# deepspeedai/DeepSpeed

Measured on AMD Instinct MI355X. Metric: tokens/sec Llama-3-8B ZeRO-3, higher is better.
Workload: dtype bf16; 1 GPU; model=llama3-8b, global_batch=8, seq_len=4096, parallelism=zero3_dp1, grad_accum=2

## Files before the change

deepspeed_amd/ops/csrc/attention.hip:

```cpp
#include <torch/extension.h>

#include "common.h"

using bf16x8_t = __attribute__((ext_vector_type(8))) short;

constexpr int KVTILE = 64;
constexpr int VT_PAD = 8;

DEV_INLINE int vtswz(int d, int kv_byte) {
  return d * ((KVTILE + VT_PAD) * 2) + (kv_byte ^ (((d >> 5) & 3) << 5));
}


using f32x16_t = __attribute__((ext_vector_type(16))) float;
#define MFMA_BF16_32x32x16 __builtin_amdgcn_mfma_f32_32x32x16_bf16

constexpr int QB5 = 32;
constexpr int QT5 = 256;
constexpr int KT5 = 64;

DEV_INLINE float half_swap(float x, int hi) {
  int i = __builtin_bit_cast(int, x);
  auto r = __builtin_amdgcn_permlane32_swap(i, i, false, false);
  return __builtin_bit_cast(float, hi ? r[0] : r[1]);
}

DEV_INLINE unsigned int cvtpk2(float lo, float hi) {
  unsigned short a = __builtin_bit_cast(unsigned short, (__bf16)lo);
  unsigned short b = __builtin_bit_cast(unsigned short, (__bf16)hi);
  return (unsigned int)a | ((unsigned int)b << 16);
}

template <int DH>
DEV_INLINE int kswz_t(int row, int byte_off) {
  return row * (DH * 2) + (byte_off ^ ((row & 7) << 4));
}

template <int DH>
__launch_bounds__(512, 2)
__global__ void flash_fwd_v5_kernel(
    const short* __restrict__ q,
    const short* __restrict__ k,
    const short* __restrict__ v,
    short* __restrict__ out,
    float* __restrict__ lse_out,
    const float* __restrict__ kvmask,
    int B, int S, int Hq, int Hk, float scale, int causal) {
  __shared__ short k_lds[2][KT5 * DH];
  __shared__ short vt_lds[DH * (KT5 + VT_PAD)];

  const int lane = threadIdx.x & 63;
  const int wave = threadIdx.x >> 6;
  const int l31 = lane & 31;
  const int hi = lane >> 5;

  constexpr int NQF = DH / 16;
  constexpr int NOT = DH / 32;

  const int qtile = blockIdx.x;
  const int bh = blockIdx.y;
  const int b = bh / Hq;
  const int h = bh % Hq;
  const int hk = h / (Hq / Hk);
  const int qbase = qtile * QT5;
  const int wave_q = qbase + wave * QB5;
  const int my_q = wave_q + l31;

  const long long qrs = (long long)Hq * DH;
  const long long kvrs = (long long)Hk * DH;
  const short* qp = q + ((long long)b * S) * qrs + h * DH;
  const short* kp = k + ((long long)b * S) * kvrs + hk * DH;
  const short* vp = v + ((long long)b * S) * kvrs + hk * DH;
  const float* mp = kvmask ? kvmask + (long long)b * S : nullptr;

  bf16x8_t qfrag[NQF];
  {
    int srow = my_q < S ? my_q : S - 1;
    const short* src = qp + (long long)srow * qrs + hi * 8;
#pragma unroll
    for (int ks = 0; ks < NQF; ++ks)
      qfrag[ks] = *reinterpret_cast<const bf16x8_t*>(src + 16 * ks);
  }

  const float sc2 = scale * 1.44269504f;
  float m_run = -INFINITY, l_run = 0.f;
  f32x16_t ot[NOT];
#pragma unroll
  for (int mt = 0; mt < NOT; ++mt)
#pragma unroll
    for (int r = 0; r < 16; ++r) ot[mt][r] = 0.f;

  const int kv_end = causal ? min(S, qbase + QT5) : S;
  const int n_tiles = (kv_end + KT5 - 1) / KT5;

  constexpr int VTPR = DH / 16;
  const int st_row = threadIdx.x / VTPR;
  const int st_c0 = (threadIdx.x % VTPR) * 16;
  constexpr int KSEGS = KT5 * DH * 2 / 1024;
  constexpr int KPASSES = (KSEGS + 7) / 8;

#define ISSUE_K(t_)                                                          \
  {                                                                          \
    int kvb_ = (t_)*KT5;                                                     \
    short* kbuf_ = k_lds[(t_)&1];                                            \
    for (int pass = 0; pass < KPASSES; ++pass) {                             \
      int seg = pass * 8 + wave;                                             \
      int linear = seg * 1024 + lane * 16;                                   \
      int row = linear / (DH * 2);                                           \
      int colbyte = linear % (DH * 2);                                       \
      int src_col = colbyte ^ ((row & 7) << 4);                              \
      int grow = kvb_ + row;                                                 \
      int srow = grow < S ? grow : S - 1;                                    \
      const short* src = kp + (long long)srow * kvrs + (src_col >> 1);       \
      __builtin_amdgcn_global_load_lds(                                      \
          reinterpret_cast<const unsigned int*>(src),                        \
          reinterpret_cast<unsigned int*>(reinterpret_cast<char*>(kbuf_) +   \
                                          seg * 1024),                       \
          16, 0, 0);                                                         \
    }                                                                        \
  }

#define LOAD_V(t_, dst_)                                                     \
  {                                                                          \
    int grow = (t_)*KT5 + st_row;                                            \
    const short* vrow = vp + (long long)grow * kvrs;                         \
    if (st_row < KT5 && grow < S) {                                          \
      dst_[0] = *reinterpret_cast<const bf16x8_t*>(vrow + st_c0);            \
      dst_[1] = *reinterpret_cast<const bf16x8_t*>(vrow + st_c0 + 8);        \
    } else {                                                                 \
      dst_[0] = bf16x8_t{0, 0, 0, 0, 0, 0, 0, 0};                            \
      dst_[1] = bf16x8_t{0, 0, 0, 0, 0, 0, 0, 0};                            \
    }                                                                        \
  }

  bf16x8_t vreg[2], vnext[2];
  ISSUE_K(0);
  LOAD_V(0, vreg);

  for (int t = 0; t < n_tiles; ++t) {
    const int kvbase = t * KT5;
    const bool has_next = (t + 1) < n_tiles;
    if (has_next) ISSUE_K(t + 1);
    if (st_row < KT5) {
      char* vbase = reinterpret_cast<char*>(vt_lds);
#pragma unroll
      for (int cc = 0; cc < 2; ++cc) {
        int col = st_c0 + cc * 8;
#pragma unroll
        for (int j = 0; j < 8; ++j)
          *reinterpret_cast<short*>(vbase + vtswz(col + j, st_row * 2)) =
              vreg[cc][j];
      }
    }
    if (has_next) LOAD_V(t + 1, vnext);
    __syncthreads();

    f32x16_t st[2];
    __builtin_amdgcn_s_setprio(1);
#pragma unroll
    for (int mt = 0; mt < 2; ++mt) {
      f32x16_t acc;
#pragma unroll
      for (int r = 0; r < 16; ++r) acc[r] = 0.f;
      int krow = 32 * mt + l31;
#pragma unroll
      for (int ks = 0; ks < NQF; ++ks) {
        bf16x8_t kf = *reinterpret_cast<const bf16x8_t*>(
            reinterpret_cast<char*>(k_lds[t & 1]) +
            kswz_t<DH>(krow, (16 * ks + hi * 8) * 2));
        acc = MFMA_BF16_32x32x16(kf, qfrag[ks], acc, 0, 0, 0);
      }
      st[mt] = acc;
    }
    __builtin_amdgcn_s_setprio(0);

    const bool btile = (causal && (kvbase + KT5 > qbase)) ||
                       (kvbase + KT5 > S) || mp != nullptr;
    float tmax = -INFINITY;
    if (btile) {
#pragma unroll
      for (int mt = 0; mt < 2; ++mt)
#pragma unroll
        for (int r = 0; r < 16; ++r) {
          float sv = st[mt][r] * sc2;
          int gkv = kvbase + 32 * mt + (r & 3) + 8 * (r >> 2) + 4 * hi;
          if (mp && gkv < S) sv += mp[gkv] * 1.44269504f;
          if ((causal && gkv > my_q) || gkv >= S) sv = -INFINITY;
          st[mt][r] = sv;
          tmax = fmaxf(tmax, sv);
        }
    } else {
#pragma unroll
      for (int mt = 0; mt < 2; ++mt)
#pragma unroll
        for (int r = 0; r < 16; ++r) {
          float sv = st[mt][r] * sc2;
          st[mt][r] = sv;
          tmax = fmaxf(tmax, sv);
        }
    }
    tmax = fmaxf(tmax, half_swap(tmax, hi));
    if (!__all(tmax - m_run <= 11.5416f)) {
      float m_new = fmaxf(m_run, tmax);
      float c = (m_run == -INFINITY) ? 0.f : __builtin_amdgcn_exp2f(m_run - m_new);
      l_run *= c;
#pragma unroll
      for (int mt = 0; mt < NOT; ++mt)
#pragma unroll
        for (int r = 0; r < 16; ++r) ot[mt][r] *= c;
      m_run = m_new;
    }
    float m_sub = m_run;
    if (btile) m_sub = (m_run == -INFINITY) ? 0.f : m_run;
    float psum = 0.f;
#pragma unroll
    for (int mt = 0; mt < 2; ++mt)
#pragma unroll
      for (int r = 0; r < 16; ++r) {
        float p = __builtin_amdgcn_exp2f(st[mt][r] - m_sub);
        st[mt][r] = p;
        psum += p;
      }
    psum += half_swap(psum, hi);
    l_run += psum;

    bf16x8_t pfrag[4];
#pragma unroll
    for (int ks = 0; ks < 4; ++ks) {
      int mt = ks >> 1, s = ks & 1;
      unsigned int wA0 = cvtpk2(st[mt][8 * s + 0], st[mt][8 * s + 1]);
      unsigned int wA1 = cvtpk2(st[mt][8 * s + 2], st[mt][8 * s + 3]);
      unsigned int wB0 = cvtpk2(st[mt][8 * s + 4], st[mt][8 * s + 5]);
      unsigned int wB1 = cvtpk2(st[mt][8 * s + 6], st[mt][8 * s + 7]);
      auto r0 = __builtin_amdgcn_permlane32_swap((int)wA0, (int)wB0,
                                                 false, false);
      auto r1 = __builtin_amdgcn_permlane32_swap((int)wA1, (int)wB1,
                                                 false, false);
      unsigned int w[4] = {(unsigned int)r0[0], (unsigned int)r1[0],
                           (unsigned int)r0[1], (unsigned int)r1[1]};
      pfrag[ks] = *reinterpret_cast<bf16x8_t*>(w);
    }

    __builtin_amdgcn_s_setprio(1);
#pragma unroll
    for (int mt = 0; mt < NOT; ++mt) {
      int drow = 32 * mt + l31;
#pragma unroll
      for (int ks = 0; ks < 4; ++ks) {
        bf16x8_t vf = *reinterpret_cast<const bf16x8_t*>(
            reinterpret_cast<char*>(vt_lds) +
            vtswz(drow, (16 * ks + hi * 8) * 2));
        ot[mt] = MFMA_BF16_32x32x16(vf, pfrag[ks], ot[mt], 0, 0, 0);
      }
    }
    __builtin_amdgcn_s_setprio(0);
    __syncthreads();
    vreg[0] = vnext[0];
    vreg[1] = vnext[1];
  }
#undef ISSUE_K
#undef LOAD_V

  if (my_q < S) {
    float inv_l = (l_run > 0.f) ? 1.f / l_run : 0.f;
    short* orow = out + ((long long)b * S + my_q) * qrs + h * DH;
#pragma unroll
    for (int mt = 0; mt < NOT; ++mt)
#pragma unroll
      for (int g = 0; g < 4; ++g) {
        int d0 = 32 * mt + 8 * g + 4 * hi;
        unsigned int w[2];
        w[0] = cvtpk2(ot[mt][4 * g + 0] * inv_l, ot[mt][4 * g + 1] * inv_l);
        w[1] = cvtpk2(ot[mt][4 * g + 2] * inv_l, ot[mt][4 * g + 3] * inv_l);
        *reinterpret_cast<unsigned long long*>(orow + d0) =
            *reinterpret_cast<unsigned long long*>(w);
      }
    if (hi == 0 && lse_out)
      lse_out[((long long)b * Hq + h) * S + my_q] =
          0.693147181f * (m_run + __log2f(fmaxf(l_run, 1e-30f)));
  }
}

void flash_check_qkv(const at::Tensor& q, const at::Tensor& k,
                     const at::Tensor& v, const char* who) {
  CHECK_ARG(q, at::kBFloat16);
  CHECK_ARG(k, at::kBFloat16);
  CHECK_ARG(v, at::kBFloat16);
  CHECK_ON(k, q);
  CHECK_ON(v, q);
  TORCH_CHECK(q.dim() == 4 && k.dim() == 4 && v.dim() == 4, who,
              ": q, k, v must be [B,S,H,D]");
  const long D = q.size(3);
  TORCH_CHECK(D == 128 || D == 64, who, ": head_dim must be 64 or 128");
  TORCH_CHECK(q.size(1) >= 1 && q.size(2) >= 1 && k.size(2) >= 1, who,
              ": empty sequence or head dimension");
  TORCH_CHECK(k.size(0) == q.size(0) && k.size(1) == q.size(1) &&
                  k.size(3) == D,
              who, ": k must be [B,S,Hk,D] with q's B, S and D");
  TORCH_CHECK(v.sizes() == k.sizes(), who, ": v must have k's shape");
  TORCH_CHECK(q.size(2) % k.size(2) == 0, who, ": GQA requires Hq % Hk == 0");
}

const float* flash_check_kvmask(const c10::optional<at::Tensor>& kvmask,
                                const at::Tensor& q) {
  if (!kvmask.has_value() || !kvmask->defined()) return nullptr;
  TORCH_CHECK(kvmask->is_cuda() && kvmask->device() == q.device() &&
                  kvmask->scalar_type() == at::kFloat &&
                  kvmask->is_contiguous() &&
                  kvmask->numel() == q.size(0) * q.size(1),
              "kvmask must be a contiguous float [B,S] tensor on q's device");
  return kvmask->data_ptr<float>();
}

std::vector<at::Tensor> flash_attn_fwd(at::Tensor q, at::Tensor k,
                                       at::Tensor v, bool causal,
                                       double scale,
                                       c10::optional<at::Tensor> kvmask) {
  flash_check_qkv(q, k, v, "flash_attn_fwd");
  int B = q.size(0), S = q.size(1), Hq = q.size(2), D = q.size(3);
  int Hk = k.size(2);
  const float* mp = flash_check_kvmask(kvmask, q);
  const float fscale =
      scale == 0.0 ? 1.0f / std::sqrt((float)D) : (float)scale;
  auto out = at::empty_like(q);
  auto lse = at::empty({B, Hq, S}, q.options().dtype(at::kFloat));
  auto stream = c10::hip::getCurrentHIPStream();
  dim3 grid((S + QT5 - 1) / QT5, B * Hq);
  if (D == 128) {
    hipLaunchKernelGGL(flash_fwd_v5_kernel<128>, grid, dim3(512), 0,
                       stream.stream(),
                       reinterpret_cast<const short*>(q.data_ptr()),
                       reinterpret_cast<const short*>(k.data_ptr()),
                       reinterpret_cast<const short*>(v.data_ptr()),
                       reinterpret_cast<short*>(out.data_ptr()),
                       lse.data_ptr<float>(), mp, B, S, Hq, Hk, fscale,
                       causal ? 1 : 0);
  } else {
    hipLaunchKernelGGL(flash_fwd_v5_kernel<64>, grid, dim3(512), 0,
                       stream.stream(),
                       reinterpret_cast<const short*>(q.data_ptr()),
                       reinterpret_cast<const short*>(k.data_ptr()),
                       reinterpret_cast<const short*>(v.data_ptr()),
                       reinterpret_cast<short*>(out.data_ptr()),
                       lse.data_ptr<float>(), mp, B, S, Hq, Hk, fscale,
                       causal ? 1 : 0);
  }
  HIP_CHECK_KERNEL();
  return {out, lse};
}
```

deepspeed_amd/ops/csrc/attention_bwd.hip:

```cpp
#include <torch/extension.h>

#include "common.h"
#include "flash_bwd_layout.h"

using bf16x8_t = __attribute__((ext_vector_type(8))) short;
using f32x4_t = __attribute__((ext_vector_type(4))) float;
using u32x4_t = __attribute__((ext_vector_type(4))) unsigned int;
using u32x2_t = __attribute__((ext_vector_type(2))) unsigned int;

#define MFMA_BF16_16x16x32 __builtin_amdgcn_mfma_f32_16x16x32_bf16

namespace bwd {

constexpr int BR = 128;
constexpr int WR = 32;
constexpr int KTW1 = 1;
constexpr int TS = 32;
static_assert(TS == bwd_layout::TS, "the image layout is for 32-row steps");
constexpr int PT = 64;

DEV_INLINE unsigned int cvtpk2(float lo, float hi) {
  unsigned short a = __builtin_bit_cast(unsigned short, (__bf16)lo);
  unsigned short b = __builtin_bit_cast(unsigned short, (__bf16)hi);
  return (unsigned int)a | ((unsigned int)b << 16);
}

template <int DH>
__launch_bounds__(256)
__global__ void bwd_preprocess(
    const short* __restrict__ dout, const short* __restrict__ out,
    const float* __restrict__ lse,
    float* __restrict__ drowP, float* __restrict__ lseP,
    int B, int S, int Sp, int Hq) {
  constexpr int PPR = DH / 8;
  const int bh = blockIdx.y;
  const int b = bh / Hq;
  const int h = bh % Hq;
  const int s0 = blockIdx.x * PT;

  for (int i = threadIdx.x; i < PT * PPR; i += 256) {
    const int row = i / PPR;
    const int c = i % PPR;
    const int s = s0 + row;
    const long long off = (((long long)b * S + s) * Hq + h) * DH + c * 8;
    u32x4_t x = {0u, 0u, 0u, 0u};
    u32x4_t o = {0u, 0u, 0u, 0u};
    if (s < S) {
      x = *reinterpret_cast<const u32x4_t*>(dout + off);
      o = *reinterpret_cast<const u32x4_t*>(out + off);
    }
    float acc = 0.f;
#pragma unroll
    for (int w = 0; w < 4; ++w)
      acc += bf2f((short)(x[w] & 0xffff)) * bf2f((short)(o[w] & 0xffff)) +
             bf2f((short)(x[w] >> 16)) * bf2f((short)(o[w] >> 16));
#pragma unroll
    for (int m = PPR / 2; m > 0; m >>= 1) acc += __shfl_xor(acc, m, WAVE);
    if (c == 0) {
      float l = 0.f;
      if (s < S) {
        l = lse[((long long)b * Hq + h) * S + s];
        if (l == -INFINITY) l = INFINITY;
      }
      drowP[((long long)b * Hq + h) * Sp + s] = acc;
      lseP[((long long)b * Hq + h) * Sp + s] = l;
    }
  }
}

DEV_INLINE void lds_dma16(const short* src, char* lds_wave_base) {
  __builtin_amdgcn_global_load_lds(
      reinterpret_cast<const unsigned int*>(src),
      reinterpret_cast<unsigned int*>(lds_wave_base), 16, 0, 0);
}

template <int DH>
DEV_INLINE void issue_rm(const short* base, long long rs, int r0, int S,
                         char* img, int sseg, int lane) {
  const int linear = sseg * 1024 + lane * 16;
  const int src_col = bwd_layout::dma_src_byte<DH>(linear);
  const int grow = r0 + bwd_layout::dma_row<DH>(linear);
  const int srow = grow < S ? grow : S - 1;
  lds_dma16(base + (long long)srow * rs + (src_col >> 1), img + sseg * 1024);
}

template <int DH>
DEV_INLINE bf16x8_t read_rm(const char* img, int row, int ks, int l4) {
  return *reinterpret_cast<const bf16x8_t*>(
      img + bwd_layout::img_off<DH>(row, (l4 * 8 + 32 * ks) * 2));
}

DEV_INLINE unsigned lds_addr(const char* p) {
  return (unsigned)(size_t)(
      (const __attribute__((address_space(3))) char*)p);
}

struct tr_frag {
  u32x2_t lo, hi;
};

template <int DH>
DEV_INLINE tr_frag issue_tr_read(unsigned img, int dt, int lane) {
  tr_frag f;
  const unsigned a0 = img + bwd_layout::tr_read_addr<DH>(lane, dt, 0);
  const unsigned a1 = img + bwd_layout::tr_read_addr<DH>(lane, dt, 1);
  asm volatile("ds_read_b64_tr_b16 %0, %1" : "=v"(f.lo) : "v"(a0) : "memory");
  asm volatile("ds_read_b64_tr_b16 %0, %1" : "=v"(f.hi) : "v"(a1) : "memory");
  return f;
}

template <int N>
DEV_INLINE void tr_wait(tr_frag& a, tr_frag& b) {
  asm volatile("s_waitcnt lgkmcnt(%4)"
               : "+v"(a.lo), "+v"(a.hi), "+v"(b.lo), "+v"(b.hi)
               : "n"(N));
}

template <int N>
DEV_INLINE void tr_wait(tr_frag& a) {
  asm volatile("s_waitcnt lgkmcnt(%2)" : "+v"(a.lo), "+v"(a.hi) : "n"(N));
}

DEV_INLINE bf16x8_t tr_operand(const tr_frag& f) {
  u32x4_t w = {f.lo[0], f.lo[1], f.hi[0], f.hi[1]};
  return __builtin_bit_cast(bf16x8_t, w);
}

DEV_INLINE bf16x8_t pack_pair(const f32x4_t& a, const f32x4_t& b) {
  u32x4_t w = {cvtpk2(a[0], a[1]), cvtpk2(a[2], a[3]), cvtpk2(b[0], b[1]),
               cvtpk2(b[2], b[3])};
  return __builtin_bit_cast(bf16x8_t, w);
}

DEV_INLINE void store4(short* p, const f32x4_t& a) {
  u32x2_t w = {cvtpk2(a[0], a[1]), cvtpk2(a[2], a[3])};
  *reinterpret_cast<u32x2_t*>(p) = w;
}

template <int NDT, int STRIDE>
DEV_INLINE void unrotate_row(f32x4_t* acc ,
                             const float* __restrict__ cr,
                             const float* __restrict__ sr) {
#pragma unroll
  for (int dt = 0; dt < NDT / 2; ++dt) {
    const f32x4_t c = *reinterpret_cast<const f32x4_t*>(cr + 16 * dt);
    const f32x4_t sn = *reinterpret_cast<const f32x4_t*>(sr + 16 * dt);
    const f32x4_t d1 = acc[dt * STRIDE];
    const f32x4_t d2 = acc[(dt + NDT / 2) * STRIDE];
    acc[dt * STRIDE] = d1 * c + d2 * sn;
    acc[(dt + NDT / 2) * STRIDE] = d2 * c - d1 * sn;
  }
}

template <int DH, int KTW, bool ROPE>
__launch_bounds__(512 / KTW, 1)
__global__ void flash_bwd_dkv_kernel(
    const short* __restrict__ q,
    const short* __restrict__ k,
    const short* __restrict__ v,
    const short* __restrict__ dout,
    const float* __restrict__ lseP,
    const float* __restrict__ drowP,
    const float* __restrict__ kvmask,
    short* __restrict__ dk,
    short* __restrict__ dv,
    const float* __restrict__ rope_cos,
    const float* __restrict__ rope_sin,
    int B, int S, int Sp, int Hq, int Hk, float scale, int causal) {
  constexpr int NKS = DH / 32;
  constexpr int NDT = DH / 16;
  constexpr int IMG = TS * DH * 2;
  constexpr int SPI = DH / 16;
  constexpr int NW = 8 / KTW;
  constexpr int WRK = 16 * KTW;
  constexpr int LD_OFF = 2 * IMG;
  constexpr int BUF = LD_OFF + 256;
  __shared__ __attribute__((aligned(16))) char smem[2 * BUF];

  const int lane = threadIdx.x & 63;
  const int wave = __builtin_amdgcn_readfirstlane(threadIdx.x >> 6);
  const int l15 = lane & 15;
  const int l4 = lane >> 4;

  const int bh = blockIdx.y;
  const int b = bh / Hk;
  const int hk = bh % Hk;
  const int G = Hq / Hk;
  const int kv_base = blockIdx.x * BR;
  const int wk = kv_base + wave * WRK;

  const long long qrs = (long long)Hq * DH;
  const long long kvrs = (long long)Hk * DH;
  const short* kp = k + ((long long)b * S) * kvrs + hk * DH;
  const short* vp = v + ((long long)b * S) * kvrs + hk * DH;

  bf16x8_t kfrag[KTW][NKS], vfrag[KTW][NKS];
  float maskv[KTW];
#pragma unroll
  for (int kt = 0; kt < KTW; ++kt) {
    const int krow = wk + 16 * kt + l15;
    const int srow = krow < S ? krow : S - 1;
    const short* ks = kp + (long long)srow * kvrs;
    const short* vs = vp + (long long)srow * kvrs;
#pragma unroll
    for (int ks_i = 0; ks_i < NKS; ++ks_i) {
      kfrag[kt][ks_i] =
          *reinterpret_cast<const bf16x8_t*>(ks + ks_i * 32 + l4 * 8);
      vfrag[kt][ks_i] =
          *reinterpret_cast<const bf16x8_t*>(vs + ks_i * 32 + l4 * 8);
    }
    maskv[kt] = (kvmask && krow < S) ? kvmask[(long long)b * S + krow] : 0.f;
  }
#pragma unroll
  for (int kt = 0; kt < KTW; ++kt) {
#pragma unroll
    for (int ks_i = 0; ks_i < NKS; ++ks_i) {
      asm volatile("" : "+v"(kfrag[kt][ks_i]));
      asm volatile("" : "+v"(vfrag[kt][ks_i]));
    }
    asm volatile("" : "+v"(maskv[kt]));
  }

  f32x4_t dk_acc[NDT][KTW], dv_acc[NDT][KTW];
#pragma unroll
  for (int dt = 0; dt < NDT; ++dt)
#pragma unroll
    for (int kt = 0; kt < KTW; ++kt) {
      dk_acc[dt][kt] = f32x4_t{0.f, 0.f, 0.f, 0.f};
      dv_acc[dt][kt] = f32x4_t{0.f, 0.f, 0.f, 0.f};
    }

  const int q_start = causal ? kv_base : 0;
  const int nq = (S - q_start + TS - 1) / TS;
  const int total = G * nq;

  static_assert(SPI <= NW, "one image segment per wave at the most");
  auto issue = [&](int g, int qb, int bufi) {
    const int h = hk * G + g;
    char* buf = smem + bufi * BUF;
    const short* qp = q + ((long long)b * S) * qrs + h * DH;
    const short* dop = dout + ((long long)b * S) * qrs + h * DH;
    const long long roff = ((long long)b * Hq + h) * Sp;
    if (wave < SPI) {
      issue_rm<DH>(qp, qrs, qb, S, buf, wave, lane);
      issue_rm<DH>(dop, qrs, qb, S, buf + IMG, wave, lane);
    }
    if (wave == 0) {
      const float* s = (lane < 32 ? lseP : drowP) + roff + qb + (lane & 31);
      __builtin_amdgcn_global_load_lds(
          reinterpret_cast<const unsigned int*>(s),
          reinterpret_cast<unsigned int*>(buf + LD_OFF), 4, 0, 0);
    }
  };

  int g_nx = 0, qb_nx = q_start;
  issue(g_nx, qb_nx, 0);
  for (int it = 0; it < total; ++it) {
    const int qb = qb_nx;
    asm volatile("s_waitcnt vmcnt(0)" ::: "memory");
    __builtin_amdgcn_s_barrier();
    asm volatile("" ::: "memory");
    qb_nx += TS;
    if (qb_nx >= S) {
      qb_nx = q_start;
      ++g_nx;
    }
    if (it + 1 < total) issue(g_nx, qb_nx, (it + 1) & 1);

    if (wk >= S || (causal && qb + TS - 1 < wk)) continue;
    const bool interior = !kvmask && qb + TS <= S && wk + WRK <= S &&
                          (!causal || qb >= wk + WRK - 1);
    const char* buf = smem + (it & 1) * BUF;
    const float* ld = reinterpret_cast<const float*>(buf + LD_OFF);

    f32x4_t s_acc[2][KTW], dp_acc[2][KTW], lrow[2];
#pragma unroll
    for (int qt = 0; qt < 2; ++qt) {
      lrow[qt] = *reinterpret_cast<const f32x4_t*>(ld + 16 * qt + 4 * l4);
      f32x4_t dr = *reinterpret_cast<const f32x4_t*>(ld + 32 + 16 * qt + 4 * l4);
#pragma unroll
      for (int kt = 0; kt < KTW; ++kt) {
        s_acc[qt][kt] = f32x4_t{0.f, 0.f, 0.f, 0.f};
        dp_acc[qt][kt] = -dr;
      }
    }
    __builtin_amdgcn_s_setprio(1);
#pragma unroll
    for (int qt = 0; qt < 2; ++qt)
#pragma unroll
      for (int ks_i = 0; ks_i < NKS; ++ks_i) {
        bf16x8_t aq = read_rm<DH>(buf, l15 + 16 * qt, ks_i, l4);
        bf16x8_t ad = read_rm<DH>(buf + IMG, l15 + 16 * qt, ks_i, l4);
#pragma unroll
        for (int kt = 0; kt < KTW; ++kt) {
          s_acc[qt][kt] = MFMA_BF16_16x16x32(aq, kfrag[kt][ks_i],
                                             s_acc[qt][kt], 0, 0, 0);
          dp_acc[qt][kt] = MFMA_BF16_16x16x32(ad, vfrag[kt][ks_i],
                                              dp_acc[qt][kt], 0, 0, 0);
        }
      }
    __builtin_amdgcn_s_setprio(0);

    if (interior) {
#pragma unroll
      for (int qt = 0; qt < 2; ++qt)
#pragma unroll
        for (int kt = 0; kt < KTW; ++kt)
#pragma unroll
          for (int r = 0; r < 4; ++r) {
            float p = __expf(s_acc[qt][kt][r] * scale - lrow[qt][r]);
            s_acc[qt][kt][r] = p;
            dp_acc[qt][kt][r] = p * dp_acc[qt][kt][r] * scale;
          }
    } else {
#pragma unroll
      for (int qt = 0; qt < 2; ++qt)
#pragma unroll
        for (int kt = 0; kt < KTW; ++kt) {
          const int gkv = wk + 16 * kt + l15;
#pragma unroll
          for (int r = 0; r < 4; ++r) {
            const int gq = qb + 16 * qt + 4 * l4 + r;
            const bool valid = gq < S && gkv < S && (!causal || gq >= gkv);
            float sval = s_acc[qt][kt][r] * scale + maskv[kt];
            float p = valid ? __expf(sval - lrow[qt][r]) : 0.f;
            s_acc[qt][kt][r] = p;
            dp_acc[qt][kt][r] = p * dp_acc[qt][kt][r] * scale;
          }
        }
    }
    bf16x8_t pb[KTW], dsb[KTW];
#pragma unroll
    for (int kt = 0; kt < KTW; ++kt) {
      pb[kt] = pack_pair(s_acc[0][kt], s_acc[1][kt]);
      dsb[kt] = pack_pair(dp_acc[0][kt], dp_acc[1][kt]);
    }

    const unsigned qimg = lds_addr(buf);
    tr_frag fq[2], fd[2];
    fq[0] = issue_tr_read<DH>(qimg, 0, lane);
    fd[0] = issue_tr_read<DH>(qimg + IMG, 0, lane);
    __builtin_amdgcn_s_setprio(1);
#pragma unroll
    for (int dt = 0; dt < NDT; ++dt) {
      if (dt + 1 < NDT) {
        fq[(dt + 1) & 1] = issue_tr_read<DH>(qimg, dt + 1, lane);
        fd[(dt + 1) & 1] = issue_tr_read<DH>(qimg + IMG, dt + 1, lane);
        tr_wait<4>(fq[dt & 1], fd[dt & 1]);
      } else {
        tr_wait<0>(fq[dt & 1], fd[dt & 1]);
      }
      const bf16x8_t aqt = tr_operand(fq[dt & 1]);
      const bf16x8_t adt = tr_operand(fd[dt & 1]);
#pragma unroll
      for (int kt = 0; kt < KTW; ++kt) {
        dv_acc[dt][kt] =
            MFMA_BF16_16x16x32(adt, pb[kt], dv_acc[dt][kt], 0, 0, 0);
        dk_acc[dt][kt] =
            MFMA_BF16_16x16x32(aqt, dsb[kt], dk_acc[dt][kt], 0, 0, 0);
      }
    }
    __builtin_amdgcn_s_setprio(0);
  }

#pragma unroll
  for (int kt = 0; kt < KTW; ++kt) {
    const int gkv = wk + 16 * kt + l15;
    if (gkv >= S) continue;
    short* dkr = dk + ((long long)b * S + gkv) * kvrs + hk * DH + 4 * l4;
    short* dvr = dv + ((long long)b * S + gkv) * kvrs + hk * DH + 4 * l4;
    if (ROPE)
      unrotate_row<NDT, KTW>(&dk_acc[0][kt],
                             rope_cos + (long long)gkv * (DH / 2) + 4 * l4,
                             rope_sin + (long long)gkv * (DH / 2) + 4 * l4);
#pragma unroll
    for (int dt = 0; dt < NDT; ++dt) {
      store4(dkr + 16 * dt, dk_acc[dt][kt]);
      store4(dvr + 16 * dt, dv_acc[dt][kt]);
    }
  }
}

template <int DH, bool ROPE>
__launch_bounds__(256, 2)
__global__ void flash_bwd_dq_kernel(
    const short* __restrict__ q, const short* __restrict__ k,
    const short* __restrict__ v, const short* __restrict__ dout,
    const float* __restrict__ lseP,
    const float* __restrict__ drowP,
    const float* __restrict__ kvmask,
    short* __restrict__ dq,
    const float* __restrict__ rope_cos,
    const float* __restrict__ rope_sin,
    int B, int S, int Sp, int Hq, int Hk, float scale, int causal) {
  constexpr int NKS = DH / 32;
  constexpr int NDT = DH / 16;
  constexpr int IMG = TS * DH * 2;
  constexpr int SPI = DH / 16;
  constexpr int IPI = SPI / 4;
  constexpr int BUF = 2 * IMG;
  __shared__ __attribute__((aligned(16))) char smem[2 * BUF];

  const int lane = threadIdx.x & 63;
  const int wave = threadIdx.x >> 6;
  const int l15 = lane & 15;
  const int l4 = lane >> 4;

  const int qtile = gridDim.x - 1 - blockIdx.x;
  const int bh = blockIdx.y;
  const int b = bh / Hq;
  const int h = bh % Hq;
  const int hk = h / (Hq / Hk);
  const int qbase = qtile * BR;
  const int wq = qbase + wave * WR;

  const long long qrs = (long long)Hq * DH;
  const long long kvrs = (long long)Hk * DH;
  const short* qp = q + ((long long)b * S) * qrs + h * DH;
  const short* dop = dout + ((long long)b * S) * qrs + h * DH;
  const short* kp = k + ((long long)b * S) * kvrs + hk * DH;
  const short* vp = v + ((long long)b * S) * kvrs + hk * DH;
  const float* mp = kvmask ? kvmask + (long long)b * S : nullptr;

  bf16x8_t qfrag[2][NKS], dofrag[2][NKS];
  float lse_l[2], dr_l[2];
#pragma unroll
  for (int qt = 0; qt < 2; ++qt) {
    const int qrow = wq + 16 * qt + l15;
    const int srow = qrow < S ? qrow : S - 1;
    const short* qs = qp + (long long)srow * qrs;
    const short* ds = dop + (long long)srow * qrs;
#pragma unroll
    for (int ks_i = 0; ks_i < NKS; ++ks_i) {
      qfrag[qt][ks_i] =
          *reinterpret_cast<const bf16x8_t*>(qs + ks_i * 32 + l4 * 8);
      dofrag[qt][ks_i] =
          *reinterpret_cast<const bf16x8_t*>(ds + ks_i * 32 + l4 * 8);
    }
    lse_l[qt] = lseP[((long long)b * Hq + h) * Sp + qrow];
    dr_l[qt] = drowP[((long long)b * Hq + h) * Sp + qrow];
  }

  f32x4_t dq_acc[NDT][2];
#pragma unroll
  for (int dt = 0; dt < NDT; ++dt)
#pragma unroll
    for (int qt = 0; qt < 2; ++qt) dq_acc[dt][qt] = f32x4_t{0.f, 0.f, 0.f, 0.f};

  const int kv_end = causal ? min(S, qbase + BR) : S;
  const int n_tiles = (kv_end + TS - 1) / TS;

  auto issue = [&](int kvb, int bufi) {
    char* buf = smem + bufi * BUF;
#pragma unroll
    for (int i = 0; i < IPI; ++i) {
      const int sseg = i * 4 + wave;
      issue_rm<DH>(kp, kvrs, kvb, S, buf, sseg, lane);
      issue_rm<DH>(vp, kvrs, kvb, S, buf + IMG, sseg, lane);
    }
  };

  issue(0, 0);
  for (int t = 0; t < n_tiles; ++t) {
    const int kvb = t * TS;
    asm volatile("s_waitcnt vmcnt(0)" ::: "memory");
    __syncthreads();
    if (t + 1 < n_tiles) issue(kvb + TS, (t + 1) & 1);

    if (wq >= S || (causal && kvb > wq + WR - 1)) continue;
    const bool interior = !mp && kvb + TS <= S && wq + WR <= S &&
                          (!causal || kvb + TS - 1 <= wq);
    const char* buf = smem + (t & 1) * BUF;

    f32x4_t s_acc[2][2], dp_acc[2][2];
#pragma unroll
    for (int kt = 0; kt < 2; ++kt)
#pragma unroll
      for (int qt = 0; qt < 2; ++qt) {
        s_acc[kt][qt] = f32x4_t{0.f, 0.f, 0.f, 0.f};
        dp_acc[kt][qt] =
            f32x4_t{-dr_l[qt], -dr_l[qt], -dr_l[qt], -dr_l[qt]};
      }
    __builtin_amdgcn_s_setprio(1);
#pragma unroll
    for (int kt = 0; kt < 2; ++kt)
#pragma unroll
      for (int ks_i = 0; ks_i < NKS; ++ks_i) {
        bf16x8_t ak = read_rm<DH>(buf, l15 + 16 * kt, ks_i, l4);
        bf16x8_t av = read_rm<DH>(buf + IMG, l15 + 16 * kt, ks_i, l4);
#pragma unroll
        for (int qt = 0; qt < 2; ++qt) {
          s_acc[kt][qt] = MFMA_BF16_16x16x32(ak, qfrag[qt][ks_i],
                                             s_acc[kt][qt], 0, 0, 0);
          dp_acc[kt][qt] = MFMA_BF16_16x16x32(av, dofrag[qt][ks_i],
                                              dp_acc[kt][qt], 0, 0, 0);
        }
      }
    __builtin_amdgcn_s_setprio(0);

    if (interior) {
#pragma unroll
      for (int kt = 0; kt < 2; ++kt)
#pragma unroll
        for (int qt = 0; qt < 2; ++qt)
#pragma unroll
          for (int r = 0; r < 4; ++r) {
            float p = __expf(s_acc[kt][qt][r] * scale - lse_l[qt]);
            dp_acc[kt][qt][r] = p * dp_acc[kt][qt][r] * scale;
          }
    } else {
#pragma unroll
      for (int kt = 0; kt < 2; ++kt)
#pragma unroll
        for (int r = 0; r < 4; ++r) {
          const int gkv = kvb + 16 * kt + 4 * l4 + r;
          const float mv = (mp && gkv < S) ? mp[gkv] : 0.f;
#pragma unroll
          for (int qt = 0; qt < 2; ++qt) {
            const int gq = wq + 16 * qt + l15;
            const bool valid = gq < S && gkv < S && (!causal || gkv <= gq);
            float sval = s_acc[kt][qt][r] * scale + mv;
            float p = valid ? __expf(sval - lse_l[qt]) : 0.f;
            dp_acc[kt][qt][r] = p * dp_acc[kt][qt][r] * scale;
          }
        }
    }
    bf16x8_t dsb[2];
#pragma unroll
    for (int qt = 0; qt < 2; ++qt)
      dsb[qt] = pack_pair(dp_acc[0][qt], dp_acc[1][qt]);

    const unsigned kimg = lds_addr(buf);
    tr_frag fk[2];
    fk[0] = issue_tr_read<DH>(kimg, 0, lane);
    __builtin_amdgcn_s_setprio(1);
#pragma unroll
    for (int dt = 0; dt < NDT; ++dt) {
      if (dt + 1 < NDT) {
        fk[(dt + 1) & 1] = issue_tr_read<DH>(kimg, dt + 1, lane);
        tr_wait<2>(fk[dt & 1]);
      } else {
        tr_wait<0>(fk[dt & 1]);
      }
      const bf16x8_t akt = tr_operand(fk[dt & 1]);
#pragma unroll
      for (int qt = 0; qt < 2; ++qt)
        dq_acc[dt][qt] =
            MFMA_BF16_16x16x32(akt, dsb[qt], dq_acc[dt][qt], 0, 0, 0);
    }
    __builtin_amdgcn_s_setprio(0);
  }

#pragma unroll
  for (int qt = 0; qt < 2; ++qt) {
    const int gq = wq + 16 * qt + l15;
    if (gq >= S) continue;
    short* dqr = dq + ((long long)b * S + gq) * qrs + h * DH + 4 * l4;
    if (ROPE)
      unrotate_row<NDT, 2>(&dq_acc[0][qt],
                           rope_cos + (long long)gq * (DH / 2) + 4 * l4,
                           rope_sin + (long long)gq * (DH / 2) + 4 * l4);
#pragma unroll
    for (int dt = 0; dt < NDT; ++dt) store4(dqr + 16 * dt, dq_acc[dt][qt]);
  }
}

}

template <int DH, bool ROPE>
static void launch_bwd(at::Tensor& q, at::Tensor& k, at::Tensor& v,
                       at::Tensor& dout, at::Tensor& out, at::Tensor& lse,
                       at::Tensor& dq, at::Tensor& dk, at::Tensor& dv,
                       const float* mp, const float* cosp, const float* sinp,
                       int B, int S, int Hq, int Hk, float scale,
                       int causal) {
  auto stream = c10::hip::getCurrentHIPStream();
  const int Sp = (S + bwd::BR - 1) / bwd::BR * bwd::BR;
  auto drow = at::empty({B, Hq, Sp}, q.options().dtype(at::kFloat));
  auto lseP = at::empty({B, Hq, Sp}, q.options().dtype(at::kFloat));
  auto sp = [](const at::Tensor& t) {
    return reinterpret_cast<const short*>(t.data_ptr());
  };
  auto spm = [](at::Tensor& t) {
    return reinterpret_cast<short*>(t.data_ptr());
  };
  dim3 grid0(Sp / bwd::PT, B * Hq);
  hipLaunchKernelGGL(bwd::bwd_preprocess<DH>, grid0, dim3(256), 0,
                     stream.stream(), sp(dout), sp(out),
                     lse.data_ptr<float>(), drow.data_ptr<float>(),
                     lseP.data_ptr<float>(), B, S, Sp, Hq);
  HIP_CHECK_KERNEL();
  dim3 grid1(Sp / bwd::BR, B * Hk);
  hipLaunchKernelGGL((bwd::flash_bwd_dkv_kernel<DH, bwd::KTW1, ROPE>), grid1,
                     dim3(512 / bwd::KTW1), 0, stream.stream(), sp(q), sp(k),
                     sp(v), sp(dout), lseP.data_ptr<float>(),
                     drow.data_ptr<float>(), mp, spm(dk), spm(dv), cosp, sinp,
                     B, S, Sp, Hq, Hk, scale, causal);
  HIP_CHECK_KERNEL();
  dim3 grid2(Sp / bwd::BR, B * Hq);
  hipLaunchKernelGGL((bwd::flash_bwd_dq_kernel<DH, ROPE>), grid2, dim3(256), 0,
                     stream.stream(), sp(q), sp(k), sp(v), sp(dout),
                     lseP.data_ptr<float>(), drow.data_ptr<float>(), mp,
                     spm(dq), cosp, sinp, B, S, Sp, Hq, Hk, scale, causal);
  HIP_CHECK_KERNEL();
}

void flash_check_qkv(const at::Tensor& q, const at::Tensor& k,
                     const at::Tensor& v, const char* who);
const float* flash_check_kvmask(const c10::optional<at::Tensor>& kvmask,
                                const at::Tensor& q);
void check_rope_table(const at::Tensor& cos, const at::Tensor& sin,
                      const at::Tensor& ref, long long S, int D,
                      const char* who);

std::vector<at::Tensor> flash_attn_bwd(at::Tensor q, at::Tensor k,
                                       at::Tensor v, at::Tensor dout,
                                       at::Tensor out, at::Tensor lse,
                                       bool causal, double scale,
                                       c10::optional<at::Tensor> kvmask,
                                       c10::optional<at::Tensor> cos,
                                       c10::optional<at::Tensor> sin) {
  flash_check_qkv(q, k, v, "flash_attn_bwd");
  CHECK_ARG(dout, at::kBFloat16);
  CHECK_ARG(out, at::kBFloat16);
  CHECK_ARG(lse, at::kFloat);
  CHECK_ON(dout, q);
  CHECK_ON(out, q);
  CHECK_ON(lse, q);
  TORCH_CHECK(dout.sizes() == q.sizes() && out.sizes() == q.sizes(),
              "flash_attn_bwd: dout and out must have q's shape");
  int B = q.size(0), S = q.size(1), Hq = q.size(2), D = q.size(3);
  int Hk = k.size(2);
  TORCH_CHECK(lse.dim() == 3 && lse.size(0) == B && lse.size(1) == Hq &&
                  lse.size(2) == S,
              "flash_attn_bwd: lse must be [B,Hq,S]");
  const float* mp = flash_check_kvmask(kvmask, q);
  const float fscale =
      scale == 0.0 ? 1.0f / std::sqrt((float)D) : (float)scale;
  auto dq = at::empty_like(q);
  auto dk = at::empty_like(k);
  auto dv = at::empty_like(v);
  TORCH_CHECK(cos.has_value() == sin.has_value(),
              "flash_attn_bwd: cos and sin must be given together");
  const bool rope = cos.has_value();
  const float* cosp = nullptr;
  const float* sinp = nullptr;
  if (rope) {
    check_rope_table(*cos, *sin, q, S, D, "flash_attn_bwd");
    cosp = cos->data_ptr<float>();
    sinp = sin->data_ptr<float>();
  }
  const int ic = causal ? 1 : 0;
#define DSAMD_LAUNCH_BWD(DH_, ROPE_)                                        \
  launch_bwd<DH_, ROPE_>(q, k, v, dout, out, lse, dq, dk, dv, mp, cosp, sinp, \
                         B, S, Hq, Hk, fscale, ic)
  if (D == 128) {
    if (rope) DSAMD_LAUNCH_BWD(128, true); else DSAMD_LAUNCH_BWD(128, false);
  } else {
    if (rope) DSAMD_LAUNCH_BWD(64, true); else DSAMD_LAUNCH_BWD(64, false);
  }
#undef DSAMD_LAUNCH_BWD
  return {dq, dk, dv};
}
```

Measured before the change: 18220 tokens/s.

## Stage V via async LDS DMA and transpose-read it for forward attention

The forward flash-attention kernel no longer loads V into registers and scatters it into a transposed LDS buffer element by element. V now goes in row-major through global_load_lds DMA, double-buffered alongside K, and is read with ds_read_b64_tr_b16 transposing loads that are software-pipelined against the PV MFMAs. The second __syncthreads per tile is also removed in favour of a single vmcnt wait plus barrier. In exchange LDS use doubles (four 16KB images), which may limit occupancy, and the shared transpose-read helpers move into a common header.

```diff
diff --git a/deepspeed_amd/ops/csrc/attention.hip b/deepspeed_amd/ops/csrc/attention.hip
--- a/deepspeed_amd/ops/csrc/attention.hip
+++ b/deepspeed_amd/ops/csrc/attention.hip
@@ -1,15 +1,10 @@
 #include <torch/extension.h>
 
 #include "common.h"
+#include "flash_fwd_layout.h"
+#include "lds_tr_read.h"
 
 using bf16x8_t = __attribute__((ext_vector_type(8))) short;
-
-constexpr int KVTILE = 64;
-constexpr int VT_PAD = 8;
-
-DEV_INLINE int vtswz(int d, int kv_byte) {
-  return d * ((KVTILE + VT_PAD) * 2) + (kv_byte ^ (((d >> 5) & 3) << 5));
-}
 
 
 using f32x16_t = __attribute__((ext_vector_type(16))) float;
@@ -31,14 +26,26 @@
   return (unsigned int)a | ((unsigned int)b << 16);
 }
 
+static_assert(KT5 == fwd_layout::KT, "the image layout is for 64-key tiles");
+
+DEV_INLINE void fwd_dma16(const short* src, char* lds_wave_base) {
+  __builtin_amdgcn_global_load_lds(
+      reinterpret_cast<const unsigned int*>(src),
+      reinterpret_cast<unsigned int*>(lds_wave_base), 16, 0, 0);
+}
+
 template <int DH>
-DEV_INLINE int kswz_t(int row, int byte_off) {
-  return row * (DH * 2) + (byte_off ^ ((row & 7) << 4));
+DEV_INLINE void issue_v_dtile(tr_frag (&f)[4], unsigned base) {
+  using namespace fwd_layout;
+  f[0] = issue_tr_read_off<v_tr_step<DH>(0, 0), v_tr_step<DH>(0, 1)>(base);
+  f[1] = issue_tr_read_off<v_tr_step<DH>(1, 0), v_tr_step<DH>(1, 1)>(base);
+  f[2] = issue_tr_read_off<v_tr_step<DH>(2, 0), v_tr_step<DH>(2, 1)>(base);
+  f[3] = issue_tr_read_off<v_tr_step<DH>(3, 0), v_tr_step<DH>(3, 1)>(base);
 }
 
 template <int DH>
 __launch_bounds__(512, 2)
-__global__ void flash_fwd_v5_kernel(
+__global__ void flash_fwd_v6_kernel(
     const short* __restrict__ q,
     const short* __restrict__ k,
     const short* __restrict__ v,
@@ -46,11 +53,11 @@
     float* __restrict__ lse_out,
     const float* __restrict__ kvmask,
     int B, int S, int Hq, int Hk, float scale, int causal) {
-  __shared__ short k_lds[2][KT5 * DH];
-  __shared__ short vt_lds[DH * (KT5 + VT_PAD)];
+  constexpr int IMG = KT5 * DH * 2;
+  __shared__ __attribute__((aligned(16))) char smem[4 * IMG];
 
   const int lane = threadIdx.x & 63;
-  const int wave = threadIdx.x >> 6;
+  const int wave = __builtin_amdgcn_readfirstlane(threadIdx.x >> 6);
   const int l31 = lane & 31;
   const int hi = lane >> 5;
 
@@ -80,6 +87,8 @@
 #pragma unroll
     for (int ks = 0; ks < NQF; ++ks)
       qfrag[ks] = *reinterpret_cast<const bf16x8_t*>(src + 16 * ks);
+#pragma unroll
+    for (int ks = 0; ks < NQF; ++ks) asm volatile("" : "+v"(qfrag[ks]));
   }
 
   const float sc2 = scale * 1.44269504f;
@@ -93,67 +102,37 @@
   const int kv_end = causal ? min(S, qbase + QT5) : S;
   const int n_tiles = (kv_end + KT5 - 1) / KT5;
 
-  constexpr int VTPR = DH / 16;
-  const int st_row = threadIdx.x / VTPR;
-  const int st_c0 = (threadIdx.x % VTPR) * 16;
-  constexpr int KSEGS = KT5 * DH * 2 / 1024;
-  constexpr int KPASSES = (KSEGS + 7) / 8;
-
-#define ISSUE_K(t_)                                                          \
-  {                                                                          \
-    int kvb_ = (t_)*KT5;                                                     \
-    short* kbuf_ = k_lds[(t_)&1];                                            \
-    for (int pass = 0; pass < KPASSES; ++pass) {                             \
-      int seg = pass * 8 + wave;                                             \
-      int linear = seg * 1024 + lane * 16;                                   \
-      int row = linear / (DH * 2);                                           \
-      int colbyte = linear % (DH * 2);                                       \
-      int src_col = colbyte ^ ((row & 7) << 4);                              \
-      int grow = kvb_ + row;                                                 \
-      int srow = grow < S ? grow : S - 1;                                    \
-      const short* src = kp + (long long)srow * kvrs + (src_col >> 1);       \
-      __builtin_amdgcn_global_load_lds(                                      \
-          reinterpret_cast<const unsigned int*>(src),                        \
-          reinterpret_cast<unsigned int*>(reinterpret_cast<char*>(kbuf_) +   \
-                                          seg * 1024),                       \
-          16, 0, 0);                                                         \
-    }                                                                        \
-  }
-
-#define LOAD_V(t_, dst_)                                                     \
-  {                                                                          \
-    int grow = (t_)*KT5 + st_row;                                            \
-    const short* vrow = vp + (long long)grow * kvrs;                         \
-    if (st_row < KT5 && grow < S) {                                          \
-      dst_[0] = *reinterpret_cast<const bf16x8_t*>(vrow + st_c0);            \
-      dst_[1] = *reinterpret_cast<const bf16x8_t*>(vrow + st_c0 + 8);        \
-    } else {                                                                 \
-      dst_[0] = bf16x8_t{0, 0, 0, 0, 0, 0, 0, 0};                            \
-      dst_[1] = bf16x8_t{0, 0, 0, 0, 0, 0, 0, 0};                            \
-    }                                                                        \
-  }
-
-  bf16x8_t vreg[2], vnext[2];
-  ISSUE_K(0);
-  LOAD_V(0, vreg);
+  constexpr int SEGS = IMG / 1024;
+  static_assert(SEGS % 8 == 0, "whole passes of the 8 waves");
+  constexpr int PASSES = SEGS / 8;
+  auto issue_tile = [&](int t_) {
+    char* kimg_ = smem + (t_ & 1) * IMG;
+    char* vimg_ = smem + (2 + (t_ & 1)) * IMG;
+#pragma unroll
+    for (int pass = 0; pass < PASSES; ++pass) {
+      const int seg = pass * 8 + wave;
+      const int linear = seg * 1024 + lane * 16;
+      const int grow = t_ * KT5 + fwd_layout::dma_row<DH>(linear);
+      const int srow = grow < S ? grow : S - 1;
+      const long long roff = (long long)srow * kvrs;
+      fwd_dma16(kp + roff + (fwd_layout::k_dma_src_byte<DH>(linear) >> 1),
+                kimg_ + seg * 1024);
+      fwd_dma16(vp + roff + (fwd_layout::v_dma_src_byte<DH>(linear) >> 1),
+                vimg_ + seg * 1024);
+    }
+  };
+
+  const unsigned smem_a = lds_addr(smem);
+  issue_tile(0);
 
   for (int t = 0; t < n_tiles; ++t) {
     const int kvbase = t * KT5;
-    const bool has_next = (t + 1) < n_tiles;
-    if (has_next) ISSUE_K(t + 1);
-    if (st_row < KT5) {
-      char* vbase = reinterpret_cast<char*>(vt_lds);
-#pragma unroll
-      for (int cc = 0; cc < 2; ++cc) {
-        int col = st_c0 + cc * 8;
-#pragma unroll
-        for (int j = 0; j < 8; ++j)
-          *reinterpret_cast<short*>(vbase + vtswz(col + j, st_row * 2)) =
-              vreg[cc][j];
-      }
-    }
-    if (has_next) LOAD_V(t + 1, vnext);
-    __syncthreads();
+    asm volatile("s_waitcnt vmcnt(0)" ::: "memory");
+    __builtin_amdgcn_s_barrier();
+    asm volatile("" ::: "memory");
+    if (t + 1 < n_tiles) issue_tile(t + 1);
+    const char* kimg = smem + (t & 1) * IMG;
+    const unsigned vimg = smem_a + (2 + (t & 1)) * IMG;
 
     f32x16_t st[2];
     __builtin_amdgcn_s_setprio(1);
@@ -162,17 +141,18 @@
       f32x16_t acc;
 #pragma unroll
       for (int r = 0; r < 16; ++r) acc[r] = 0.f;
-      int krow = 32 * mt + l31;
 #pragma unroll
       for (int ks = 0; ks < NQF; ++ks) {
         bf16x8_t kf = *reinterpret_cast<const bf16x8_t*>(
-            reinterpret_cast<char*>(k_lds[t & 1]) +
-            kswz_t<DH>(krow, (16 * ks + hi * 8) * 2));
+            kimg + fwd_layout::k_row_read_addr<DH>(lane, mt, ks));
         acc = MFMA_BF16_32x32x16(kf, qfrag[ks], acc, 0, 0, 0);
       }
       st[mt] = acc;
     }
     __builtin_amdgcn_s_setprio(0);
+
+    tr_frag vf[2][4];
+    issue_v_dtile<DH>(vf[0], vimg + fwd_layout::v_tr_lane_base<DH>(lane, 0));
 
     const bool btile = (causal && (kvbase + KT5 > qbase)) ||
                        (kvbase + KT5 > S) || mp != nullptr;
@@ -244,22 +224,21 @@
     __builtin_amdgcn_s_setprio(1);
 #pragma unroll
     for (int mt = 0; mt < NOT; ++mt) {
-      int drow = 32 * mt + l31;
-#pragma unroll
-      for (int ks = 0; ks < 4; ++ks) {
-        bf16x8_t vf = *reinterpret_cast<const bf16x8_t*>(
-            reinterpret_cast<char*>(vt_lds) +
-            vtswz(drow, (16 * ks + hi * 8) * 2));
-        ot[mt] = MFMA_BF16_32x32x16(vf, pfrag[ks], ot[mt], 0, 0, 0);
+      if (mt + 1 < NOT) {
+        issue_v_dtile<DH>(
+            vf[(mt + 1) & 1],
+            vimg + fwd_layout::v_tr_lane_base<DH>(lane, mt + 1));
+        tr_wait<8>(vf[mt & 1]);
+      } else {
+        tr_wait<0>(vf[mt & 1]);
       }
+#pragma unroll
+      for (int ks = 0; ks < 4; ++ks)
+        ot[mt] = MFMA_BF16_32x32x16(tr_operand(vf[mt & 1][ks]), pfrag[ks],
+                                    ot[mt], 0, 0, 0);
     }
     __builtin_amdgcn_s_setprio(0);
-    __syncthreads();
-    vreg[0] = vnext[0];
-    vreg[1] = vnext[1];
   }
-#undef ISSUE_K
-#undef LOAD_V
 
   if (my_q < S) {
     float inv_l = (l_run > 0.f) ? 1.f / l_run : 0.f;
@@ -327,7 +306,7 @@
   auto stream = c10::hip::getCurrentHIPStream();
   dim3 grid((S + QT5 - 1) / QT5, B * Hq);
   if (D == 128) {
-    hipLaunchKernelGGL(flash_fwd_v5_kernel<128>, grid, dim3(512), 0,
+    hipLaunchKernelGGL(flash_fwd_v6_kernel<128>, grid, dim3(512), 0,
                        stream.stream(),
                        reinterpret_cast<const short*>(q.data_ptr()),
                        reinterpret_cast<const short*>(k.data_ptr()),
@@ -336,7 +315,7 @@
                        lse.data_ptr<float>(), mp, B, S, Hq, Hk, fscale,
                        causal ? 1 : 0);
   } else {
-    hipLaunchKernelGGL(flash_fwd_v5_kernel<64>, grid, dim3(512), 0,
+    hipLaunchKernelGGL(flash_fwd_v6_kernel<64>, grid, dim3(512), 0,
                        stream.stream(),
                        reinterpret_cast<const short*>(q.data_ptr()),
                        reinterpret_cast<const short*>(k.data_ptr()),
diff --git a/deepspeed_amd/ops/csrc/attention_bwd.hip b/deepspeed_amd/ops/csrc/attention_bwd.hip
--- a/deepspeed_amd/ops/csrc/attention_bwd.hip
+++ b/deepspeed_amd/ops/csrc/attention_bwd.hip
@@ -2,6 +2,7 @@
 
 #include "common.h"
 #include "flash_bwd_layout.h"
+#include "lds_tr_read.h"
 
 using bf16x8_t = __attribute__((ext_vector_type(8))) short;
 using f32x4_t = __attribute__((ext_vector_type(4))) float;
@@ -90,40 +91,10 @@
       img + bwd_layout::img_off<DH>(row, (l4 * 8 + 32 * ks) * 2));
 }
 
-DEV_INLINE unsigned lds_addr(const char* p) {
-  return (unsigned)(size_t)(
-      (const __attribute__((address_space(3))) char*)p);
-}
-
-struct tr_frag {
-  u32x2_t lo, hi;
-};
-
 template <int DH>
 DEV_INLINE tr_frag issue_tr_read(unsigned img, int dt, int lane) {
-  tr_frag f;
-  const unsigned a0 = img + bwd_layout::tr_read_addr<DH>(lane, dt, 0);
-  const unsigned a1 = img + bwd_layout::tr_read_addr<DH>(lane, dt, 1);
-  asm volatile("ds_read_b64_tr_b16 %0, %1" : "=v"(f.lo) : "v"(a0) : "memory");
-  asm volatile("ds_read_b64_tr_b16 %0, %1" : "=v"(f.hi) : "v"(a1) : "memory");
-  return f;
-}
-
-template <int N>
-DEV_INLINE void tr_wait(tr_frag& a, tr_frag& b) {
-  asm volatile("s_waitcnt lgkmcnt(%4)"
-               : "+v"(a.lo), "+v"(a.hi), "+v"(b.lo), "+v"(b.hi)
-               : "n"(N));
-}
-
-template <int N>
-DEV_INLINE void tr_wait(tr_frag& a) {
-  asm volatile("s_waitcnt lgkmcnt(%2)" : "+v"(a.lo), "+v"(a.hi) : "n"(N));
-}
-
-DEV_INLINE bf16x8_t tr_operand(const tr_frag& f) {
-  u32x4_t w = {f.lo[0], f.lo[1], f.hi[0], f.hi[1]};
-  return __builtin_bit_cast(bf16x8_t, w);
+  return ::issue_tr_read(img + bwd_layout::tr_read_addr<DH>(lane, dt, 0),
+                       img + bwd_layout::tr_read_addr<DH>(lane, dt, 1));
 }
 
 DEV_INLINE bf16x8_t pack_pair(const f32x4_t& a, const f32x4_t& b) {
diff --git a/deepspeed_amd/ops/csrc/flash_fwd_layout.h b/deepspeed_amd/ops/csrc/flash_fwd_layout.h
--- /dev/null
+++ b/deepspeed_amd/ops/csrc/flash_fwd_layout.h
@@ -0,0 +1,73 @@
+#pragma once
+
+#if defined(__HIPCC__)
+#define FFL_HD __host__ __device__ __forceinline__
+#else
+#define FFL_HD inline
+#endif
+
+namespace fwd_layout {
+
+constexpr int KT = 64;
+
+template <int DH>
+FFL_HD int v_xor(int row) {
+  constexpr int RB = DH * 2;
+  constexpr int RPB = 256 / RB;
+  constexpr int NU = RB / 64;
+  return ((row / RPB) & (NU - 1)) << 6;
+}
+
+template <int DH>
+FFL_HD int k_xor(int row) {
+  constexpr int RB = DH * 2;
+  constexpr int RPB = 256 / RB;
+  constexpr int NC = RB / 16;
+  return ((row / RPB) & (NC - 1)) << 4;
+}
+
+template <int DH>
+FFL_HD int v_off(int row, int byte_off) {
+  return row * (DH * 2) + (byte_off ^ v_xor<DH>(row));
+}
+template <int DH>
+FFL_HD int k_off(int row, int byte_off) {
+  return row * (DH * 2) + (byte_off ^ k_xor<DH>(row));
+}
+
+template <int DH>
+FFL_HD int dma_row(int linear) {
+  return linear / (DH * 2);
+}
+template <int DH>
+FFL_HD int v_dma_src_byte(int linear) {
+  return (linear % (DH * 2)) ^ v_xor<DH>(dma_row<DH>(linear));
+}
+template <int DH>
+FFL_HD int k_dma_src_byte(int linear) {
+  return (linear % (DH * 2)) ^ k_xor<DH>(dma_row<DH>(linear));
+}
+
+template <int DH>
+FFL_HD int k_row_read_addr(int lane, int mt, int ks) {
+  const int l31 = lane & 31, hi = lane >> 5;
+  return k_off<DH>(32 * mt + l31, (16 * ks + 8 * hi) * 2);
+}
+
+template <int DH>
+FFL_HD int v_tr_lane_base(int lane, int mt) {
+  const int l15 = lane & 15, g = lane >> 4;
+  const int hi = g >> 1, dh = g & 1;
+  const int q = l15 >> 2, p = l15 & 3;
+  return v_off<DH>(8 * hi + q, 64 * mt + 32 * dh + 8 * p);
+}
+template <int DH>
+FFL_HD constexpr int v_tr_step(int ks, int hf) {
+  return (16 * ks + 4 * hf) * (DH * 2);
+}
+template <int DH>
+FFL_HD int v_tr_read_addr(int lane, int mt, int ks, int hf) {
+  return v_tr_lane_base<DH>(lane, mt) + v_tr_step<DH>(ks, hf);
+}
+
+}
diff --git a/deepspeed_amd/ops/csrc/lds_tr_read.h b/deepspeed_amd/ops/csrc/lds_tr_read.h
--- /dev/null
+++ b/deepspeed_amd/ops/csrc/lds_tr_read.h
@@ -0,0 +1,60 @@
+#pragma once
+
+#include "common.h"
+
+using lds_u32x4_t = __attribute__((ext_vector_type(4))) unsigned int;
+using lds_u32x2_t = __attribute__((ext_vector_type(2))) unsigned int;
+using lds_bf16x8_t = __attribute__((ext_vector_type(8))) short;
+
+DEV_INLINE unsigned lds_addr(const char* p) {
+  return (unsigned)(size_t)(
+      (const __attribute__((address_space(3))) char*)p);
+}
+
+struct tr_frag {
+  lds_u32x2_t lo, hi;
+};
+
+DEV_INLINE tr_frag issue_tr_read(unsigned a0, unsigned a1) {
+  tr_frag f;
+  asm volatile("ds_read_b64_tr_b16 %0, %1" : "=v"(f.lo) : "v"(a0) : "memory");
+  asm volatile("ds_read_b64_tr_b16 %0, %1" : "=v"(f.hi) : "v"(a1) : "memory");
+  return f;
+}
+
+template <int OFF0, int OFF1>
+DEV_INLINE tr_frag issue_tr_read_off(unsigned base) {
+  static_assert(OFF0 >= 0 && OFF0 < 65536 && OFF1 >= 0 && OFF1 < 65536,
+                "ds offset field is 16 bits");
+  tr_frag f;
+  asm volatile("ds_read_b64_tr_b16 %0, %1 offset:%2"
+               : "=v"(f.lo) : "v"(base), "n"(OFF0) : "memory");
+  asm volatile("ds_read_b64_tr_b16 %0, %1 offset:%2"
+               : "=v"(f.hi) : "v"(base), "n"(OFF1) : "memory");
+  return f;
+}
+
+template <int N>
+DEV_INLINE void tr_wait(tr_frag& a, tr_frag& b) {
+  asm volatile("s_waitcnt lgkmcnt(%4)"
+               : "+v"(a.lo), "+v"(a.hi), "+v"(b.lo), "+v"(b.hi)
+               : "n"(N));
+}
+
+template <int N>
+DEV_INLINE void tr_wait(tr_frag& a) {
+  asm volatile("s_waitcnt lgkmcnt(%2)" : "+v"(a.lo), "+v"(a.hi) : "n"(N));
+}
+
+template <int N>
+DEV_INLINE void tr_wait(tr_frag (&f)[4]) {
+  asm volatile("s_waitcnt lgkmcnt(%8)"
+               : "+v"(f[0].lo), "+v"(f[0].hi), "+v"(f[1].lo), "+v"(f[1].hi),
+                 "+v"(f[2].lo), "+v"(f[2].hi), "+v"(f[3].lo), "+v"(f[3].hi)
+               : "n"(N));
+}
+
+DEV_INLINE lds_bf16x8_t tr_operand(const tr_frag& f) {
+  lds_u32x4_t w = {f.lo[0], f.lo[1], f.hi[0], f.hi[1]};
+  return __builtin_bit_cast(lds_bf16x8_t, w);
+}
```

Result: faster. 18610 tokens/s, median of 6 (+2.1%).
